# Ryukhaan/speech-to-video-mpp

Measured on AMD Instinct MI355X. Metric: synthesized 256×256 frames/sec/GPU (LNet+ENet path); 1/2/4/8-GPU scaling, higher is better.
Workload: dtype f32; 1 GPU; ENet(+LNet) forward, B=16 synthetic 256x256 crops + [1,80,16] mel windows -> 384x384 (models/ENet.py:82-139); crop=256, global_batch=16, batch_per_gpu=16, parallelism=frame-shard x1 (no data-path collective), graph=True, lanes=1, world_size_seen=1

## Files before the change

include/s2v.h:

```cpp
#ifndef S2V_H_
#define S2V_H_

#include <stddef.h>
#include <stdint.h>

#ifdef __cplusplus
extern "C" {
#endif

typedef void *s2v_stream_t;

enum {
    S2V_OK = 0,
    S2V_E_INVALID = -1,
    S2V_E_LAUNCH = -2,
    S2V_E_WORKSPACE = -3
};

enum {
    S2V_ACT_NONE = 0,
    S2V_ACT_RELU = 1,
    S2V_ACT_LRELU = 2,
    S2V_ACT_SIGMOID = 3,
    S2V_ACT_TANH = 4,
// ... 86 lines not shown

int s2v_modconv_demod_rows(const float *s, int batch, int s_ns, const int *rows, int nrows,
                           const float *wsq, float eps, float post, float *d, int d_ns,
                           s2v_stream_t stream);

int s2v_resize(const float *x, int n, int c, int ih, int iw, long long xsn, long long xsc, long long xsy,
               long long xsx, float *y, int oh, int ow, long long ysn, long long ysc, long long ysy,
               long long ysx, float scale_h, float scale_w, int mode, s2v_stream_t stream);

int s2v_torgb_up2(const float *x, int n, int h, int w, int c, int xcs, const float *wt, int kpad, const float *s,
                  int s_ns, const float *bias, const float *skip, int skcs, float *y, int ycs, s2v_stream_t stream);

typedef struct s2v_torgb_win {
    int fh, fw;
    int oy, ox;
    int sh, sw;
    int sy, sx;
    int nchw, cy, cx;
} s2v_torgb_win;
int s2v_torgb_up2_win(const float *x, int n, int h, int w, int c, int xcs, const float *wt, int kpad, const float *s,
                      int s_ns, const float *bias, const float *skip, int skcs, float *y, int ycs,
                      const s2v_torgb_win *win, s2v_stream_t stream);

typedef struct s2v_tapsum_win {
    int fh, fw;
    int oy, ox;
    int sy, sx;
} s2v_tapsum_win;
int s2v_tapsum_up2(const float *p, int n, int ph, int pw, int pcs, int cout, const float *noise, float pix_w,
                   const float *bias, float gain, int act, float alpha, float *y, int oh, int ow, int ycs,
                   const s2v_tapsum_win *win, s2v_stream_t stream);

int s2v_row_pack(const float *x, int n, int h, int w, int c, int xcs, int kw, int pw, float *y, int ycs,
                 s2v_stream_t stream);

int s2v_pad_reflect(const float *x, int n, int h, int w, int c, int xcs, int pt, int pb, int pl, int pr,
                    float *y, int ycs, s2v_stream_t stream);

int s2v_row_layernorm(const float *x, int rows, int dim, int xld, const float *weight, const float *bias,
                      float eps, float *y, int yld, s2v_stream_t stream);

int s2v_attention(const float *q, const float *k, const float *v, int batch, int heads, int tokens,
                  int dim_head, int ld_q, int ld_k, int ld_v, long long bs_q, long long bs_k, long long bs_v,
                  float scale, float *o, int ld_o, long long bs_o, s2v_stream_t stream);

int s2v_flow_warp(const float *flow, int n, int fh, int fw, int flow_cs, const float *src, int c, int h,
                  int w, long long ssn, long long ssc, long long ssy, long long ssx, float *y, int ycs,
                  s2v_stream_t stream);
int s2v_flow_warp_cat(const float *flow, int n, int fh, int fw, int flow_cs, const float *src, int c, int h,
                      int w, long long ssn, long long ssc, long long ssy, long long ssx, float *y, int ycs,
// ... 196 lines not shown
```

speech-to-video-mpp_amd/csrc/torch_launch.cpp:

```cpp
#include <ATen/ATen.h>
#include <ATen/hip/HIPContext.h>
#include <c10/core/DeviceGuard.h>
#include <torch/library.h>

#include <vector>

#include "../../include/s2v.h"

namespace {

using at::Tensor;
using OptT = c10::optional<Tensor>;

void *stream() { return (void *)at::hip::getCurrentHIPStream().stream(); }

void check(int rc, const char *what) { TORCH_CHECK(rc == 0, what, " failed (", rc, "): ", s2v_last_error()); }

bool has(const OptT &t) { return t && t->defined(); }

void same_dev(const Tensor &t, const at::Device &dev, const char *what) {
    TORCH_CHECK(t.is_cuda(), what, ": expected a HIP device tensor (the s2v ops have no CPU kernel)");
    TORCH_CHECK(t.device() == dev, what, ": on ", t.device(), ", the op's inputs are on ", dev);
}

// ... 677 lines not shown
        win.sy = (int)window[4]; win.sx = (int)window[5];
    }
    float *yp = nullptr;
    int ycs = 0;
    if (crop.empty()) {
        const NV yv = nhwc(y, dev, "torgb y");
        TORCH_CHECK(yv.n == xv.n && yv.h == xv.h && yv.w == xv.w && yv.c == 4, "torgb: y [N, H, W, 4] view expected");
        yp = yv.p; ycs = yv.cs;
    } else {
        f32(y, dev, "torgb y");
        TORCH_CHECK(crop[0] >= 0 && crop[1] >= 0 && 2 * crop[0] < xv.h && 2 * crop[1] < xv.w, "torgb crop: bad (cy, cx)");
        win.nchw = 1; win.cy = (int)crop[0]; win.cx = (int)crop[1];
        TORCH_CHECK(y.dim() == 4 && y.is_contiguous() && y.size(0) == xv.n && y.size(1) == 3 &&
                        y.size(2) == xv.h - 2 * win.cy && y.size(3) == xv.w - 2 * win.cx,
                    "torgb: contiguous NCHW y [N, 3, H - 2 cy, W - 2 cx] expected, got ", y.sizes());
        yp = y.data_ptr<float>();
    }
    check(s2v_torgb_up2_win(xv.p, xv.n, xv.h, xv.w, xv.c, xv.cs, wt.data_ptr<float>(), (int)wt.size(1),
                            s.data_ptr<float>(), s_ns, bp, kv.p, kv.cs, yp, ycs, &win, stream()),
          "s2v_torgb_up2");
}

void tapsum_up2_(const Tensor &p, const OptT &noise, double pix_w, const OptT &bias, double gain, int64_t act,
                 double alpha, const Tensor &y, at::IntArrayRef window) {
    const c10::DeviceGuard guard(p.device());
    const at::Device dev = p.device();
    const NV pv = nhwc(p, dev, "tapsum p"), yv = nhwc(y, dev, "tapsum y");
    TORCH_CHECK(yv.n == pv.n && pv.c == 9 * yv.c, "tapsum: p [N, PH, PW, 9 C] and y [N, OH, OW, C] views expected");
    TORCH_CHECK(window.empty() || window.size() == 6, "tapsum window: (fh, fw, oy, ox, sy, sx) or empty");
    s2v_tapsum_win win{};
    if (window.empty()) {
        TORCH_CHECK(yv.h == 2 * pv.h && yv.w == 2 * pv.w, "tapsum: y [N, 2 PH, 2 PW, C] expected");
    } else {
        for (int64_t v : window) TORCH_CHECK(v >= 0 && v < (1 << 29), "tapsum window: bad value ", v);
        win.fh = (int)window[0]; win.fw = (int)window[1]; win.oy = (int)window[2]; win.ox = (int)window[3];
        win.sy = (int)window[4]; win.sx = (int)window[5];
    }
    const float *np = vec(noise, dev, (int64_t)yv.n * yv.h * yv.w, "tapsum noise");
    const float *bp = vec(bias, dev, yv.c, "tapsum bias");
    check(s2v_tapsum_up2(pv.p, pv.n, pv.h, pv.w, pv.cs, yv.c, np, (float)pix_w, bp, (float)gain, (int)act, (float)alpha,
                         yv.p, yv.h, yv.w, yv.cs, &win, stream()),
          "s2v_tapsum_up2");
}

void flow_warp_(const Tensor &flow, const Tensor &src, const Tensor &y) {
    const c10::DeviceGuard guard(flow.device());
    const at::Device dev = flow.device();
    const NV fv = nhwc(flow, dev, "flow_warp flow"), yv = nhwc(y, dev, "flow_warp y");
    f32(src, dev, "flow_warp src");
    TORCH_CHECK(src.dim() == 4 && src.size(0) == fv.n && fv.c >= 2, "flow_warp: src [N, C, H, W], flow >= 2 channels");
    TORCH_CHECK(yv.n == fv.n && yv.h == src.size(2) && yv.w == src.size(3) && yv.c == src.size(1), "flow_warp: y shape");
    check(s2v_flow_warp(fv.p, fv.n, fv.h, fv.w, fv.cs, src.data_ptr<float>(), (int)src.size(1), (int)src.size(2),
                        (int)src.size(3), src.stride(0), src.stride(1), src.stride(2), src.stride(3), yv.p, yv.cs,
                        stream()),
          "s2v_flow_warp");
}

void flow_warp_cat_(const Tensor &flow, const Tensor &src, const Tensor &y) {
    const c10::DeviceGuard guard(flow.device());
    const at::Device dev = flow.device();
// ... 299 lines not shown
    m.def("group_end_(Tensor? ws, bool dry) -> int[]", &group_end_);
    m.def("gemm_kn_(Tensor a, Tensor b, Tensor(a!) out, int batch, int a_bs, int b_bs, int out_bs, Tensor? res, "
          "int res_bs, int act, float alpha, int prec, Tensor? ws, int force_tile, int force_splits, bool dry) -> int[]");
    m.def("split_weights_(Tensor w, Tensor(a!) out, int prec, float scale) -> ()");
    m.def("split_act_(Tensor x, Tensor(a!) out, int prec) -> ()");
    m.def("layernorm2d_(Tensor x, Tensor weight, Tensor bias, float eps, int act, float alpha, bool pool, "
          "Tensor? res, Tensor(a!) y, Tensor? ws) -> int");
    m.def("instnorm_(Tensor x, Tensor? gamma, Tensor? beta, float eps, int act, float alpha, Tensor? res, "
          "Tensor(a!) y, Tensor(b!)? pad_out, Tensor? ws) -> int");
    m.def("adain_params_(Tensor hid, int nhidden, Tensor w2t, Tensor bias, Tensor seg, Tensor(a!) out) -> ()");
    m.def("modconv_demod_(Tensor s, Tensor wsq, Tensor(a!) d, float eps, float post) -> ()");
    m.def("modconv_demod_rows_(Tensor s, Tensor rows, Tensor wsq, Tensor(a!) d, float eps, float post, "
          "int s_reach) -> ()");
    m.def("row_layernorm_(Tensor x, Tensor weight, Tensor bias, float eps, Tensor(a!) y) -> ()");
    m.def("attention_(Tensor q, Tensor k, Tensor v, Tensor(a!) out, int batch, int heads, int tokens, int dim_head, "
          "float scale) -> ()");
    m.def("resize_(Tensor x, int x_off, int[4] x_size, int[4] x_stride, Tensor(a!) y, int y_off, int[4] y_size, "
          "int[4] y_stride, float scale_h, float scale_w, int mode) -> ()");
    m.def("pad_reflect_(Tensor x, Tensor(a!) y, int[4] pads) -> ()");
    m.def("row_pack_(Tensor x, Tensor(a!) y, int kw, int pw) -> ()");
    m.def("torgb_up2_(Tensor x, Tensor wt, Tensor s, Tensor? bias, Tensor skip, Tensor(a!) y, int[] window, "
          "int[] crop) -> ()");
    m.def("tapsum_up2_(Tensor p, Tensor? noise, float pix_w, Tensor? bias, float gain, int act, float alpha, "
          "Tensor(a!) y, int[] window) -> ()");
    m.def("flow_warp_(Tensor flow, Tensor src, Tensor(a!) y) -> ()");
    m.def("flow_warp_cat_(Tensor flow, Tensor src, Tensor(a!) y) -> ()");
    m.def("fill_value_(Tensor(a!) y, float value) -> ()");
    m.def("gaussian_noise_(Tensor(a!) y, int seed, int offset, Tensor? ctr, int shift) -> ()");
    m.def("counter_add_(Tensor(a!) ctr, int inc) -> ()");
    m.def("rfft2_(Tensor x, Tensor tables, Tensor(a!) spec) -> ()");
    m.def("irfft2_(Tensor spec, Tensor tables, Tensor? res, Tensor(a!) y) -> ()");
    m.def("ffc_spec_fwd_(Tensor x_g, Tensor w1, float wt_scale, float x_scale, Tensor? scale, Tensor? shift, "
          "Tensor tables, Tensor(a!) t1, Tensor(b!) spec, Tensor? flag, int prec) -> ()");
    m.def("ffc_spec_inv_(Tensor spec, Tensor wfu, float wt_scale, float x_scale, Tensor? scale, Tensor? shift, "
          "Tensor tables, Tensor t1, Tensor(a!) u, Tensor? flag, int prec) -> ()");
    m.def("ffc_norm_(Tensor(c!) y, Tensor u, Tensor w2, float wt_scale, float x_scale, Tensor? gamma, Tensor? beta, "
          "float eps, int act, float alpha, Tensor? res, Tensor(a!) out, Tensor(b!)? pad_out, Tensor? flag, int prec) -> ()");
    m.def("eltwise_(Tensor x, Tensor? mul, Tensor? add, Tensor? bias, float a, int act, float alpha, float post, "
          "Tensor(a!) y) -> ()");
    m.def("fir2d_(Tensor x, Tensor kernel, Tensor(a!) y, int up, int down, int pad_y0, int pad_x0, float gain, "
          "Tensor? bias, int act, float alpha, float post) -> ()");
    m.def("lipsync_inputs_(Tensor src, Tensor? fake, Tensor(a!) ref_u8, Tensor(b!) face6, Tensor(c!) gt) -> ()");
    m.def("to_u8_(Tensor x, Tensor(a!) y, float lo, float hi, float scale, float offset) -> ()");
    m.def("mel_chunks_(Tensor mel, Tensor starts, int step, Tensor(a!) out) -> ()");
    m.def("melspectrogram_(Tensor wav, Tensor tables, bool pad_reflect, Tensor(a!) out) -> ()");
}

// ... 38 lines not shown
```

speech-to-video-mpp_amd/csrc/torgb.hip:

```cpp
#include "common.hpp"

namespace s2v {

__host__ __device__ __forceinline__ void up2_index(int dst, int in, int &i0, int &i1, float &l0, float &l1) {
    float src = 0.5f * ((float)dst + 0.5f) - 0.5f;
    if (src < 0.f) src = 0.f;
    i0 = (int)src;
    i1 = i0 + ((i0 < in - 1) ? 1 : 0);
    l1 = src - (float)i0;
    l0 = 1.f - l1;
}


struct TorgbGeo {
    int fsh, fsw;
    int oy, ox;
    int sh, sw;
    int sy, sx;
    int nchw, cy, cx;
};

template <int TPP, int PPT>
__global__ __launch_bounds__(256) void torgb_up2_kernel(const float *__restrict__ x, int C, int H, int W, int xcs,
                                                        const float *__restrict__ wt, int kpad,
// ... 97 lines not shown
    hi = i1;
}

struct TapsumGeo {
    int fh, fw;
    int ph, pw, sy, sx;
    int oh, ow, oy, ox;
    int k0, j0, ckh, ckw;
};

struct TapsumEpi {
    const float *noise;
    float pix_w;
    const float *bias;
    float gain;
    int act;
    float alpha;
    float *y;
    int ycs;
};

__device__ __forceinline__ constexpr float tapsum_w(int par, int ti) { return (par ^ ti) ? 0.25f : 0.75f; }

template <int DY, int DX>
__device__ __forceinline__ void tapsum_tap(const float *__restrict__ pt, const long long (&ro)[3], const long long (&co)[3],
                                           float4 (&acc)[2][2]) {
    constexpr int kLo[3] = {0, 0, 1}, kHi[3] = {1, 2, 2};
    float4 v[3][3];
#pragma unroll
    for (int si = 0; si < 3; ++si)
#pragma unroll
        for (int sj = 0; sj < 3; ++sj)
            if (si >= kLo[DY] && si <= kHi[DY] && sj >= kLo[DX] && sj <= kHi[DX])
                v[si][sj] = *(const float4 *)(pt + ro[si] + co[sj]);
#pragma unroll
    for (int a = 0; a < 2; ++a)
#pragma unroll
        for (int c = 0; c < 2; ++c) {
            const int bi = a + DY <= 1 ? 0 : 1, bj = c + DX <= 1 ? 0 : 1;
#pragma unroll
            for (int ti = 0; ti < 2; ++ti)
#pragma unroll
                for (int tj = 0; tj < 2; ++tj) {
                    const float cf = tapsum_w((a + DY) & 1, ti) * tapsum_w((c + DX) & 1, tj);
                    const float4 u = v[bi + ti][bj + tj];
                    acc[a][c].x = fmaf(cf, u.x, acc[a][c].x);
                    acc[a][c].y = fmaf(cf, u.y, acc[a][c].y);
                    acc[a][c].z = fmaf(cf, u.z, acc[a][c].z);
                    acc[a][c].w = fmaf(cf, u.w, acc[a][c].w);
                }
        }
}

__device__ __forceinline__ void tapsum_store(const TapsumEpi &e, const TapsumGeo &g, int b, int wr, int wc, int quad,
                                             float4 acc) {
    const long long pix = ((long long)b * g.oh + wr) * g.ow + wc;
    float4 bv = make_float4(0.f, 0.f, 0.f, 0.f);
    if (e.bias) bv = *(const float4 *)(e.bias + quad * 4);
    const float nz = e.noise ? e.pix_w * e.noise[pix] : 0.f;
    float4 r;
    r.x = apply_act(e.gain * acc.x + bv.x + nz, e.act, e.alpha);
    r.y = apply_act(e.gain * acc.y + bv.y + nz, e.act, e.alpha);
    r.z = apply_act(e.gain * acc.z + bv.z + nz, e.act, e.alpha);
    r.w = apply_act(e.gain * acc.w + bv.w + nz, e.act, e.alpha);
    *(float4 *)(e.y + pix * e.ycs + quad * 4) = r;
}

__global__ __launch_bounds__(256) void tapsum_up2_kernel(const float *__restrict__ P, int pcs, int cout, int quads,
                                                         long long items, TapsumEpi e, TapsumGeo g) {
    const long long item = (long long)xcd_block(blockIdx.x, gridDim.x) * 256 + threadIdx.x;
    if (item >= items) return;
    const int quad = (int)(item % quads);
    long long cell = item / quads;
    const int cj = (int)(cell % g.ckw);
    cell /= g.ckw;
    const int ck = (int)(cell % g.ckh);
    const int b = (int)(cell / g.ckh);
    const int k = g.k0 + ck, j = g.j0 + cj;
    const float *pb = P + (long long)b * g.ph * g.pw * pcs + quad * 4;
    if (k >= 1 && k <= g.fh - 2 && j >= 1 && j <= g.fw - 2) {
        long long ro[3], co[3];
#pragma unroll
        for (int s = 0; s < 3; ++s) {
            ro[s] = (long long)min(max(k + s - 1 - g.sy, 0), g.ph - 1) * g.pw * pcs;
            co[s] = (long long)min(max(j + s - 1 - g.sx, 0), g.pw - 1) * pcs;
        }
        float4 acc[2][2];
#pragma unroll
        for (int a = 0; a < 2; ++a)
#pragma unroll
            for (int c = 0; c < 2; ++c) acc[a][c] = make_float4(0.f, 0.f, 0.f, 0.f);
#pragma unroll 1
        for (int t = 0; t < 9; ++t) {
            const float *pt = pb + t * cout;
            switch (t) {
                case 0: tapsum_tap<0, 0>(pt, ro, co, acc); break;
                case 1: tapsum_tap<0, 1>(pt, ro, co, acc); break;
                case 2: tapsum_tap<0, 2>(pt, ro, co, acc); break;
                case 3: tapsum_tap<1, 0>(pt, ro, co, acc); break;
                case 4: tapsum_tap<1, 1>(pt, ro, co, acc); break;
                case 5: tapsum_tap<1, 2>(pt, ro, co, acc); break;
                case 6: tapsum_tap<2, 0>(pt, ro, co, acc); break;
                case 7: tapsum_tap<2, 1>(pt, ro, co, acc); break;
                default: tapsum_tap<2, 2>(pt, ro, co, acc); break;
            }
        }
#pragma unroll
        for (int a = 0; a < 2; ++a)
#pragma unroll
            for (int c = 0; c < 2; ++c) {
                const int wr = 2 * k + a - g.oy, wc = 2 * j + c - g.ox;
                if ((unsigned)wr < (unsigned)g.oh && (unsigned)wc < (unsigned)g.ow) tapsum_store(e, g, b, wr, wc, quad, acc[a][c]);
            }
        return;
    }
#pragma unroll 1
    for (int ac = 0; ac < 4; ++ac) {
        const int r = 2 * k + (ac >> 1), c = 2 * j + (ac & 1);
        const int wr = r - g.oy, wc = c - g.ox;
        if ((unsigned)wr >= (unsigned)g.oh || (unsigned)wc >= (unsigned)g.ow) continue;
        float4 acc = make_float4(0.f, 0.f, 0.f, 0.f);
#pragma unroll 1
        for (int t = 0; t < 9; ++t) {
            const int qy = r + t / 3 - 1, qx = c + t % 3 - 1;
            int i0, i1, j0, j1;
            float ly[2], lx[2];
            up2_index(qy, g.fh, i0, i1, ly[0], ly[1]);
            up2_index(qx, g.fw, j0, j1, lx[0], lx[1]);
            if (qy < 0 || qy >= 2 * g.fh) ly[0] = ly[1] = 0.f;
            if (qx < 0 || qx >= 2 * g.fw) lx[0] = lx[1] = 0.f;
            const long long rr[2] = {(long long)min(max(i0 - g.sy, 0), g.ph - 1) * g.pw * pcs,
                                     (long long)min(max(i1 - g.sy, 0), g.ph - 1) * g.pw * pcs};
            const long long cc[2] = {(long long)min(max(j0 - g.sx, 0), g.pw - 1) * pcs,
                                     (long long)min(max(j1 - g.sx, 0), g.pw - 1) * pcs};
            const float *pt = pb + t * cout;
#pragma unroll
            for (int ti = 0; ti < 2; ++ti)
#pragma unroll
                for (int tj = 0; tj < 2; ++tj) {
                    const float cf = ly[ti] * lx[tj];
                    const float4 u = *(const float4 *)(pt + rr[ti] + cc[tj]);
                    acc.x = fmaf(cf, u.x, acc.x);
                    acc.y = fmaf(cf, u.y, acc.y);
                    acc.z = fmaf(cf, u.z, acc.z);
                    acc.w = fmaf(cf, u.w, acc.w);
                }
        }
        tapsum_store(e, g, b, wr, wc, quad, acc);
    }
}

}

using namespace s2v;

extern "C" int s2v_tapsum_up2(const float *p, int n, int ph, int pw, int pcs, int cout, const float *noise, float pix_w,
                              const float *bias, float gain, int act, float alpha, float *y, int oh, int ow, int ycs,
                              const s2v_tapsum_win *win, s2v_stream_t stream) {
    S2V_REQUIRE(p && y && win && n > 0 && ph > 0 && pw > 0 && oh > 0 && ow > 0 && cout > 0, "tapsum_up2: bad args");
    S2V_REQUIRE(cout % 4 == 0, "tapsum_up2: Cout %d must be a multiple of 4 (16-byte channel accesses)", cout);
    S2V_REQUIRE(act == S2V_ACT_NONE || act == S2V_ACT_LRELU || act == S2V_ACT_RELU, "tapsum_up2: unknown act %d", act);
    const int fh = win->fh > 0 ? win->fh : ph, fw = win->fw > 0 ? win->fw : pw;
    S2V_REQUIRE(fh < (1 << 29) && fw < (1 << 29), "tapsum_up2: frame too large");
    S2V_REQUIRE(win->oy >= 0 && win->ox >= 0 && win->oy + (long long)oh <= 2LL * fh && win->ox + (long long)ow <= 2LL * fw,
                "tapsum_up2: the %dx%d output window at (%d, %d) leaves the %dx%d frame", oh, ow, win->oy, win->ox,
                2 * fh, 2 * fw);
    S2V_REQUIRE(win->sy >= 0 && win->sx >= 0 && win->sy + (long long)ph <= fh && win->sx + (long long)pw <= fw,
                "tapsum_up2: the %dx%d tap-product window at (%d, %d) leaves the %dx%d frame", ph, pw, win->sy, win->sx,
                fh, fw);
    int ylo, yhi, xlo, xhi;
    {
        const int qy0 = win->oy > 0 ? win->oy - 1 : 0, qy1 = win->oy + oh < 2 * fh ? win->oy + oh : 2 * fh - 1;
        const int qx0 = win->ox > 0 ? win->ox - 1 : 0, qx1 = win->ox + ow < 2 * fw ? win->ox + ow : 2 * fw - 1;
        up2_tap_range(qy0, qy1 - qy0 + 1, fh, ylo, yhi);
        up2_tap_range(qx0, qx1 - qx0 + 1, fw, xlo, xhi);
    }
    S2V_REQUIRE(ylo >= win->sy && yhi < win->sy + ph && xlo >= win->sx && xhi < win->sx + pw,
                "tapsum_up2: the output window at (%d, %d) reads tap-product rows %d..%d, columns %d..%d: outside the "
                "%dx%d tap-product window at (%d, %d)", win->oy, win->ox, ylo, yhi, xlo, xhi, ph, pw, win->sy, win->sx);
    S2V_REQUIRE(pcs % 4 == 0 && pcs >= 9LL * cout && ycs % 4 == 0 && ycs >= cout,
                "tapsum_up2: pixel pitches must hold 9 Cout / Cout channels and be multiples of 4");
    S2V_REQUIRE(((uintptr_t)p % 16) == 0 && ((uintptr_t)y % 16) == 0 && (!bias || ((uintptr_t)bias % 16) == 0),
                "tapsum_up2: 16-byte aligned p / y / bias");
    S2V_REQUIRE((long long)n * ph * pw * pcs < (1LL << 62) && (long long)n * oh * ow < (1LL << 40),
                "tapsum_up2: problem too large");
    const int k0 = win->oy >> 1, j0 = win->ox >> 1;
    const int ckh = ((win->oy + oh - 1) >> 1) - k0 + 1, ckw = ((win->ox + ow - 1) >> 1) - j0 + 1;
    const int quads = cout / 4;
    const long long items = (long long)n * ckh * ckw * quads;
    const long long blocks = (items + 255) / 256;
    S2V_REQUIRE(blocks < (1LL << 31), "tapsum_up2: grid too large");
    const TapsumGeo g{fh, fw, ph, pw, win->sy, win->sx, oh, ow, win->oy, win->ox, k0, j0, ckh, ckw};
    const TapsumEpi e{noise, noise ? pix_w : 0.f, bias, gain, act, alpha, y, ycs};
    tapsum_up2_kernel<<<(unsigned)blocks, 256, 0, (hipStream_t)stream>>>(p, pcs, cout, quads, items, e, g);
    return check_launch("tapsum_up2");
}

extern "C" int s2v_torgb_up2_win(const float *x, int n, int h, int w, int c, int xcs, const float *wt, int kpad,
                                 const float *s, int s_ns, const float *bias, const float *skip, int skcs, float *y,
                                 int ycs, const s2v_torgb_win *win, s2v_stream_t stream) {
    S2V_REQUIRE(x && wt && s && skip && y && win && n > 0 && h > 1 && w > 1 && c > 0, "torgb_up2: bad args");
    const int fh = win->fh > 0 ? win->fh : h, fw = win->fw > 0 ? win->fw : w;
    S2V_REQUIRE(fh % 2 == 0 && fw % 2 == 0, "torgb_up2: output frame %dx%d must be twice the skip frame", fh, fw);
    S2V_REQUIRE(win->oy >= 0 && win->ox >= 0 && win->oy + h <= fh && win->ox + w <= fw,
                "torgb_up2: the %dx%d output window at (%d, %d) leaves the %dx%d frame", h, w, win->oy, win->ox, fh, fw);
    S2V_REQUIRE(win->sh > 0 && win->sw > 0 && win->sy >= 0 && win->sx >= 0 && win->sy + win->sh <= fh / 2 &&
                    win->sx + win->sw <= fw / 2,
                "torgb_up2: the %dx%d skip window at (%d, %d) leaves the %dx%d skip frame", win->sh, win->sw, win->sy,
                win->sx, fh / 2, fw / 2);
    int ylo, yhi, xlo, xhi;
    up2_tap_range(win->oy, h, fh / 2, ylo, yhi);
    up2_tap_range(win->ox, w, fw / 2, xlo, xhi);
    S2V_REQUIRE(ylo >= win->sy && yhi < win->sy + win->sh && xlo >= win->sx && xhi < win->sx + win->sw,
                "torgb_up2: the output window at (%d, %d) reads skip rows %d..%d, columns %d..%d: outside the %dx%d "
                "skip window at (%d, %d)", win->oy, win->ox, ylo, yhi, xlo, xhi, win->sh, win->sw, win->sy, win->sx);
    S2V_REQUIRE(c % 32 == 0 && xcs % 4 == 0 && xcs >= c && kpad >= c && s_ns >= c && skcs % 4 == 0 && skcs >= 4,
                "torgb_up2: C %% 32 == 0, 4-channel skip, float4 pitches required");
// ... 37 lines not shown
```

speech-to-video-mpp_amd/engine/enet.py:

```python
from __future__ import annotations

import math
import os

import torch

from .. import ops
from ..ops import NHWC, ConvW
from .lnet import LNetEngine

LRELU = 0.2
OVERLAP = os.environ.get("S2V_ENET_OVERLAP", "1") == "1"
FUSED_TORGB = os.environ.get("S2V_ENET_FUSED_TORGB", "1") == "1"
POLY_UP = os.environ.get("S2V_ENET_POLY_UP", "1") == "1"
POLY_UP4 = os.environ.get("S2V_ENET_POLY_UP4", "0") == "1"
STYLE_GRID = os.environ.get("S2V_ENET_STYLE_GRID", "half")
ROWPACK0 = os.environ.get("S2V_ENET_ROWPACK0", "0") == "1"
FORK_AT = int(os.environ.get("S2V_ENET_FORK_AT", "0"))
PAUSE = tuple(int(v) for v in os.environ.get("S2V_ENET_PAUSE", "").split(":")) if os.environ.get("S2V_ENET_PAUSE") else None
PREMOD = os.environ.get("S2V_ENET_PREMOD", "1") == "1"
STACK_STRIPS = os.environ.get("S2V_ENET_STACK_STRIPS", "1") == "1"
RESUME_GRID = os.environ.get("S2V_ENET_RESUME_GRID", "")
CROP_TAIL = os.environ.get("S2V_ENET_CROP_TAIL", "1") == "1"
TAPSUM = os.environ.get("S2V_ENET_TAPSUM", "1") == "1"
TAP_TILE = int(os.environ.get("S2V_ENET_TAP_TILE", "9"))
OUT_CROP = 8


def crop_tail_cone(size: int, crop: int):
    f1, f2 = 2 * size, 4 * size
    lo, hi = crop, f2 - 1 - crop
    if crop < 3 or lo > hi:
        return None
    need = {"rgb1": (lo, hi), "conv4": (lo, hi), "conv3": (lo - 1, hi + 1)}
    p0, p1 = (lo - 1) // 2, (hi + 1) // 2
    need["conv2"] = (p0 - 1, p1 + 1)
    need["conv1"] = (p0 - 2, p1 + 2)
    need["rgb0"] = ((2 * lo - 1) // 4, (2 * hi - 1) // 4 + 1)
    win = {"conv1": (1, f1 - 2), "conv2": (2, f1 - 4), "rgb0": (2, f1 - 4), "conv3": (6, f2 - 12),
           "conv4": (7, f2 - 14), "rgb1": (7, f2 - 14)}
    for k, (a, b) in need.items():
        o, n = win[k]
        if n <= 0 or a < o or b > o + n - 1:
            return None
    return {"need": need, "win": win, "crop": crop - 7, "out": f2 - 2 * crop}


def style_grid(device) -> int:
# ... 177 lines not shown
                  (cur.t[:, :, 0:2], lambda t: t[:, :, 0:4], lambda t: t[:, :, 0:2], lambda t: t[:, :, 0:2]),
                  (cur.t[:, :, cur.w - 2:], lambda t: t[:, :, w2 - 4:], lambda t: t[:, :, 2:4],
                   lambda t: t[:, :, w2 - 2:]))
        for xs_t, nsel, ssel, ysel in strips:
            xs = NHWC(xs_t.contiguous())
            up = NHWC.empty(b, 2 * xs.h, 2 * xs.w, c, dev)
            ops.resize_nhwc(ctx, xs, up, scale_factor=2)
            ys = NHWC.empty(b, up.h, up.w, L.cout, dev)
            nz = None if noise is None else nsel(noise).contiguous()
            ops.modulated_conv2d(ctx, up, L.conv, ys, s, d, pix_add=nz, premod=wb.get("conv"), **kw)
            ysel(y.t).copy_(ssel(ys.t))
        return y

    def _crop_cone(self, size, out):
        L = self.layers
        if not (CROP_TAIL and POLY_UP and FUSED_TORGB) or L[0].conv4 is not None or L[0].rp is not None or \
                L[3].conv4 is None or L[1].conv4 is not None or L[4].conv4 is not None or L[2].cin % 32 or L[5].cin % 32:
            return None
        cone = crop_tail_cone(size, OUT_CROP)
        if cone is not None and tuple(out.shape[1:]) != (3, cone["out"], cone["out"]):
            return None
        return cone

    def _noise_window(self, ctx, L, idx, b, frame, origin, n, noises, ctr):
        if not L.noise_w:
            return None
        if noises is not None and noises[idx] is not None:
            plane = noises[idx].reshape(b, frame, frame)
        else:
            plane = torch.empty((b, frame, frame), device=self.device)
            ops.gaussian_noise(ctx, plane, self.noise_seed, idx << 36, ctr=ctr, shift=40)
            self.last_noises[idx] = plane
        return plane[:, origin: origin + n, origin: origin + n].contiguous()

    def _cropped_tail(self, ctx, cur: NHWC, s2, dtab, dall, wbs, noises, ctr, out, cone):
        dev, b, win = self.device, cur.n, cone["win"]
        f1, f2 = 2 * cur.h, 4 * cur.h
        L = self.layers
        kw = dict(act=ops.ACT_LRELU, alpha=LRELU, padding=(0, 0))

        def mod(j):
            sv = s2[:, self.mod_offs[j]: self.mod_offs[j] + L[j].cin]
            if L[j].is_rgb:
                return sv, None, {}
            idx = j - j // 3
            return sv, dtab.r0[idx], wbs.get(idx, {})

        x = NHWC.empty(b, f1, f1, cur.c, dev)
        ops.resize_nhwc(ctx, cur, x, scale_factor=2)
        for j, name in ((0, "conv1"), (1, "conv2")):
            o, n = win[name]
            s, r0, wb = mod(j)
            y = NHWC.empty(b, n, n, L[j].cout, dev)
            ops.modulated_conv2d(ctx, x, L[j].conv, y, s, dall[:, r0: r0 + L[j].cout], pix_w=L[j].noise_w or 0.0,
                                 pix_add=self._noise_window(ctx, L[j], j, b, f1, o, n, noises, ctr),
                                 premod=wb.get("conv"), **kw)
            x = y
        o, n = win["rgb0"]
        rgb0 = NHWC.empty(b, n, n, 4, dev)
        ops.torgb_up2(ctx, x, L[2].conv, mod(2)[0], cur, rgb0, frame=(f1, f1), origin=(o, o))
        o3, n3 = win["conv3"]
        s, r0, wb = mod(3)
        y = NHWC.empty(b, n3, n3, L[3].cout, dev)
        nz3 = self._noise_window(ctx, L[3], 2, b, f2, o3, n3, noises, ctr)
        if TAPSUM and L[3].conv9 is not None:
            o2 = win["conv2"][0]
            self._tapsum_styleconv(ctx, L[3], x, s, dall[:, r0: r0 + dtab.width[2]], wb.get("conv9"), nz3, y,
                                   frame=(f1, f1), origin=(o3, o3), src_origin=(o2, o2))
        else:
            ops.modulated_conv2d(ctx, x, L[3].conv4, y, s, dall[:, r0: r0 + dtab.width[2]], d2s=True,
                                 pix_w=L[3].noise_w or 0.0, pix_add=nz3, premod=wb.get("conv4"), **kw)
        o4, n4 = win["conv4"]
        s, r0, wb = mod(4)
        z = NHWC.empty(b, n4, n4, L[4].cout, dev)
        ops.modulated_conv2d(ctx, y, L[4].conv, z, s, dall[:, r0: r0 + L[4].cout], pix_w=L[4].noise_w or 0.0,
                             pix_add=self._noise_window(ctx, L[4], 3, b, f2, o4, n4, noises, ctr),
                             premod=wb.get("conv"), **kw)
        dst = out if out.is_contiguous() else torch.empty(out.shape, device=dev)
        ops.torgb_up2(ctx, z, L[5].conv, mod(5)[0], rgb0, dst, frame=(f2, f2), origin=(o4, o4), skip_origin=(o, o),
                      crop=(cone["crop"], cone["crop"]))
        if dst is not out:
            out.copy_(dst)

    def style_code(self, ctx, ref: torch.Tensor):
        st = self.style_begin(ctx, ref)
        self.style_down(ctx, st, len(self.down))
        return self.style_end(ctx, st)

    def style_begin(self, ctx, ref: torch.Tensor) -> dict:
        dev, b = self.device, ref.shape[0]
        x = NHWC.empty(b, 256, 256, 4, dev)
        ops.fill(ctx, x.t)
        ops.nchw_to_nhwc(ctx, ref, x.slice(0, 3))
        f = NHWC.empty(b, 256, 256, self.first.cout, dev)
        ops.conv2d(ctx, x, self.first, f, act=ops.ACT_LRELU, alpha=LRELU)
        return {"f": f, "i": 0}

    def style_down(self, ctx, st: dict, upto: int):
        f, b, dev = st["f"], st["f"].n, self.device
# ... 4 lines not shown
            ops.conv2d(ctx, f, c1, td, act=ops.ACT_LRELU, alpha=LRELU, pool=True)
            out = NHWC.empty(b, h // 2, w // 2, c2.cout, dev)
            ops.conv2d(ctx, f, sk, out)
            ops.conv2d(ctx, td, c2, out, act=ops.ACT_LRELU, alpha=LRELU, res=out, res_after=True)
            f = out
            st["i"] += 1
        st["f"] = f

    def style_end(self, ctx, st: dict):
        f, b, dev = st["f"], st["f"].n, self.device
        g = NHWC.empty(b, f.h, f.w, self.final_conv.cout, dev)
        ops.conv2d(ctx, f, self.final_conv, g, act=ops.ACT_LRELU, alpha=LRELU)
        style = NHWC.empty(b, 1, 1, self.final_linear.cout, dev)
        ops.conv2d(ctx, NHWC(g.t.view(b, 1, 1, -1)), self.final_linear, style)
        return style

    def forward(self, ctx, audio, face, gt, out: torch.Tensor, low: torch.Tensor, noises=None, aux=None):
        dev = self.device
        b = audio.shape[0]
        svec = NHWC.empty(b, 1, 1, self.mod.cout, dev)
        side = self._side(ctx) if OVERLAP else None
        cone = self._crop_cone(96 + 4, out)
        enc = {}

        def finish(sctx):
            enc["style"] = self.style_end(sctx, enc.pop("st"))
            ops.conv2d(sctx, enc["style"], self.mod, svec)
            enc["d"] = self._demods(sctx, svec.t.view(b, -1))
            if PREMOD:
                enc["wb"] = self._premodulate(sctx, svec.t.view(b, -1), enc["d"][0], enc["d"][1], b,
                                              strips=cone is None)

        def fork():
            sst, sctx = side
            sst.wait_stream(torch.cuda.current_stream(dev))
            with ops.x3_grid_cap(sctx, style_grid(dev)), ops.side_stream(sst, ctx.keep):
                enc["st"] = self.style_begin(sctx, face[:, 3:])
                self.style_down(sctx, enc["st"], PAUSE[0] if PAUSE else len(self.down))
                if not PAUSE:
                    finish(sctx)

        def resume():
            sst, sctx = side
            sst.wait_stream(torch.cuda.current_stream(dev))
            grid = int(RESUME_GRID) if RESUME_GRID else style_grid(dev)
            with ops.x3_grid_cap(sctx, grid), ops.side_stream(sst, ctx.keep):
                self.style_down(sctx, enc["st"], len(self.down))
                finish(sctx)

        on_level = None
        if side is not None:
            if FORK_AT:
                on_level = lambda h: fork() if h == FORK_AT and not enc else None
            else:
# ... 5 lines not shown
            ops.conv2d(ctx, enc["style"], self.mod, svec)
            enc["d"] = self._demods(ctx, svec.t.view(b, -1))
        x6 = NHWC.empty(b, 96, 96, 6, dev)
        ops.nchw_to_nhwc(ctx, face[:, :3], x6.slice(0, 3))
        ops.nchw_to_nhwc(ctx, gt, x6.slice(3, 3))
        lo = NHWC.empty(b, 96, 96, 4, dev)
        self.lnet.forward(ctx, audio, x6, lo, pad_rgb=True, on_level=on_level)
        if side is not None and not enc:
            fork()
        if side is not None and "st" in enc:
            resume()
        ops.nhwc_to_nchw(ctx, lo.slice(0, 3), low)
        if side is not None:
            torch.cuda.current_stream(dev).wait_stream(side[0])
        style, (dtab, dall) = enc["style"], enc["d"]
        s2 = svec.t.view(b, -1)
        if aux is not None:
            aux["style"] = style.t.view(b, -1)
        cur = NHWC.empty(b, 100, 100, 4, dev)
        ops.pad_reflect(ctx, lo, cur, (2, 2, 2, 2))
        skip = cur
        ctr = None
        self.last_noises = [None] * 4
        if noises is None and any(L.noise_w for L in self.layers):
            ctr = ctx.noise(id(self)).bump(ctx)
        if cone is not None:
            self._cropped_tail(ctx, cur, s2, dtab, dall, enc.get("wb", {}), noises, ctr, out, cone)
            return out, low
        for st in range(2):
            for li in range(2):
                L = self.layers[3 * st + li]
                off = self.mod_offs[3 * st + li]
                r0, wd = dtab.r0[2 * st + li], dtab.width[2 * st + li]
                if POLY_UP and L.conv4 is not None:
                    cur = self._poly_styleconv(ctx, L, cur, s2[:, off: off + L.cin], dall[:, r0: r0 + wd],
                                               2 * st + li, noises, ctr, wb=enc.get("wb", {}).get(2 * st + li))
                    continue
                x = cur
                if L.upsample:
                    x = NHWC.empty(b, 2 * cur.h, 2 * cur.w, cur.c, dev)
                    ops.resize_nhwc(ctx, cur, x, scale_factor=2)
                conv, cin = L.conv, L.cin
                if L.rp is not None:
                    xp = NHWC.empty(b, x.h, x.w, L.rp, dev)
                    ops.row_pack(ctx, x, xp, L.k, L.k // 2)
                    x, conv, cin = xp, L.conv.rowpack, L.rp
                d = dall[:, r0: r0 + L.cout]
                y = NHWC.empty(b, x.h, x.w, L.cout, dev)
                noise = None
                if L.noise_w:
# ... 22 lines not shown
```

speech-to-video-mpp_amd/ops.py:

```python
from __future__ import annotations

import contextlib
import ctypes
import math
import os
import threading
import weakref

import torch

from . import _lib, torch_ops
from ._lib import (ACT_GELU_TANH, ACT_LRELU, ACT_NONE, ACT_RELU, ACT_SIGMOID, ACT_TANH,
                   IN_DIRECT, IN_NEAREST_UP2, IN_TRANSPOSED, PAD_REFLECT, PAD_ZERO, PREC_BF16X3, PREC_F16, PREC_F16X3, PREC_F32,
                   check)

F32 = 4

_PRECISIONS = {"f16x3": PREC_F16X3, "bf16x3": PREC_BF16X3, "f32": PREC_F32, "f16": PREC_F16}
SPLIT_PRECISIONS = ("f16x3", "bf16x3")
PRECISION = os.environ.get("S2V_PRECISION", "f16x3")
if PRECISION not in _PRECISIONS:
    raise ValueError(f"S2V_PRECISION must be one of {sorted(_PRECISIONS)}, got {PRECISION!r}")


# ... 888 lines not shown
    assert skip.n == x.n and skip.c == 4
    if frame is None:
        assert origin == (0, 0) and skip_origin == (0, 0) and (2 * skip.h, 2 * skip.w) == (x.h, x.w)
        window = []
    else:
        window = [int(frame[0]), int(frame[1]), int(origin[0]), int(origin[1]), int(skip_origin[0]), int(skip_origin[1])]
    if crop is None:
        assert (y.n, y.h, y.w, y.c) == (x.n, x.h, x.w, 4)
        S2V.torgb_up2_(x.v, cw.wt, s, cw.shift, skip.v, y.v, window, [])
    else:
        assert tuple(y.shape) == (x.n, 3, x.h - 2 * crop[0], x.w - 2 * crop[1])
        S2V.torgb_up2_(x.v, cw.wt, s, cw.shift, skip.v, y, window, [int(crop[0]), int(crop[1])])
    return y


def up2_tap_window(origin: int, size: int, frame: int):
    q0, q1 = max(origin - 1, 0), min(origin + size, 2 * frame - 1)
    lo = int(max(0.5 * (q0 + 0.5) - 0.5, 0.0))
    hi = min(int(max(0.5 * (q1 + 0.5) - 0.5, 0.0)) + 1, frame - 1)
    return lo, hi - lo + 1


def tapsum_up2(ctx: Ctx, p: NHWC, y: NHWC, *, bias=None, pix_add=None, pix_w=0.0, gain=1.0, act=ACT_NONE, alpha=0.0,
               frame=None, origin=(0, 0), src_origin=(0, 0)):
    assert p.n == y.n and p.c == 9 * y.c, "tapsum_up2: p carries nine tap blocks of y's channels"
    if frame is None:
        assert origin == (0, 0) and src_origin == (0, 0) and (y.h, y.w) == (2 * p.h, 2 * p.w)
        window = []
    else:
        window = [int(frame[0]), int(frame[1]), int(origin[0]), int(origin[1]), int(src_origin[0]), int(src_origin[1])]
    if pix_add is not None:
        assert tuple(pix_add.shape) == (y.n, y.h, y.w) and pix_add.is_contiguous()
    S2V.tapsum_up2_(p.v, pix_add, float(pix_w), bias, float(gain), int(act), float(alpha), y.v, window)
    return y


def row_pack(ctx: Ctx, x: NHWC, y: NHWC, kw: int, pw: int):
    S2V.row_pack_(x.v, y.v, kw, pw)
    return y


def pad_reflect(ctx: Ctx, x: NHWC, y: NHWC, pads):
    S2V.pad_reflect_(x.v, y.v, list(pads))
    return y


def row_layernorm(ctx: Ctx, x: torch.Tensor, weight, bias, y: torch.Tensor, eps=1e-5):
    S2V.row_layernorm_(x, weight, bias, eps, y)
    return y


def attention(ctx: Ctx, q: torch.Tensor, k: torch.Tensor, v: torch.Tensor, out: torch.Tensor, *, batch, heads,
              tokens, dim_head=64, scale=None):
    scale = dim_head ** -0.5 if scale is None else scale
    S2V.attention_(q, k, v, out, batch, heads, tokens, dim_head, scale)
    return out
# ... 148 lines not shown
```

Before: 741.0 frames/s.

## Compute two tapsum cells per thread and pre-draw noise planes on side stream

The tapsum upsample kernel now lets each thread process a run of two adjacent cells. The overlapping column loads of the 3x3 source neighbourhood are shared between them, which cuts redundant global loads and index math but raises register use. A separate change draws the gaussian noise planes and their cropped windows during the overlapped side-stream encode phase, moving that work off the main critical path. The cost is extra allocations and full-plane generation before cropping.

```diff
diff --git a/include/s2v.h b/include/s2v.h
--- a/include/s2v.h
+++ b/include/s2v.h
@@ -132,10 +132,13 @@
                       int s_ns, const float *bias, const float *skip, int skcs, float *y, int ycs,
                       const s2v_torgb_win *win, s2v_stream_t stream);
 
+#define S2V_TAPSUM_RUN 0
+#define S2V_TAPSUM_CELL 1
 typedef struct s2v_tapsum_win {
     int fh, fw;
     int oy, ox;
     int sy, sx;
+    int variant;
 } s2v_tapsum_win;
 int s2v_tapsum_up2(const float *p, int n, int ph, int pw, int pcs, int cout, const float *noise, float pix_w,
                    const float *bias, float gain, int act, float alpha, float *y, int oh, int ow, int ycs,
diff --git a/speech-to-video-mpp_amd/csrc/torch_launch.cpp b/speech-to-video-mpp_amd/csrc/torch_launch.cpp
--- a/speech-to-video-mpp_amd/csrc/torch_launch.cpp
+++ b/speech-to-video-mpp_amd/csrc/torch_launch.cpp
@@ -723,7 +723,7 @@
 }
 
 void tapsum_up2_(const Tensor &p, const OptT &noise, double pix_w, const OptT &bias, double gain, int64_t act,
-                 double alpha, const Tensor &y, at::IntArrayRef window) {
+                 double alpha, const Tensor &y, at::IntArrayRef window, int64_t variant) {
     const c10::DeviceGuard guard(p.device());
     const at::Device dev = p.device();
     const NV pv = nhwc(p, dev, "tapsum p"), yv = nhwc(y, dev, "tapsum y");
@@ -737,6 +737,8 @@
         win.fh = (int)window[0]; win.fw = (int)window[1]; win.oy = (int)window[2]; win.ox = (int)window[3];
         win.sy = (int)window[4]; win.sx = (int)window[5];
     }
+    TORCH_CHECK(variant >= 0 && variant <= 1, "tapsum variant: bad value ", variant);
+    win.variant = (int)variant;
     const float *np = vec(noise, dev, (int64_t)yv.n * yv.h * yv.w, "tapsum noise");
     const float *bp = vec(bias, dev, yv.c, "tapsum bias");
     check(s2v_tapsum_up2(pv.p, pv.n, pv.h, pv.w, pv.cs, yv.c, np, (float)pix_w, bp, (float)gain, (int)act, (float)alpha,
@@ -1082,7 +1084,7 @@
     m.def("torgb_up2_(Tensor x, Tensor wt, Tensor s, Tensor? bias, Tensor skip, Tensor(a!) y, int[] window, "
           "int[] crop) -> ()");
     m.def("tapsum_up2_(Tensor p, Tensor? noise, float pix_w, Tensor? bias, float gain, int act, float alpha, "
-          "Tensor(a!) y, int[] window) -> ()");
+          "Tensor(a!) y, int[] window, int variant) -> ()");
     m.def("flow_warp_(Tensor flow, Tensor src, Tensor(a!) y) -> ()");
     m.def("flow_warp_cat_(Tensor flow, Tensor src, Tensor(a!) y) -> ()");
     m.def("fill_value_(Tensor(a!) y, float value) -> ()");
diff --git a/speech-to-video-mpp_amd/csrc/torgb.hip b/speech-to-video-mpp_amd/csrc/torgb.hip
--- a/speech-to-video-mpp_amd/csrc/torgb.hip
+++ b/speech-to-video-mpp_amd/csrc/torgb.hip
@@ -143,17 +143,8 @@
 
 __device__ __forceinline__ constexpr float tapsum_w(int par, int ti) { return (par ^ ti) ? 0.25f : 0.75f; }
 
-template <int DY, int DX>
-__device__ __forceinline__ void tapsum_tap(const float *__restrict__ pt, const long long (&ro)[3], const long long (&co)[3],
-                                           float4 (&acc)[2][2]) {
-    constexpr int kLo[3] = {0, 0, 1}, kHi[3] = {1, 2, 2};
-    float4 v[3][3];
-#pragma unroll
-    for (int si = 0; si < 3; ++si)
-#pragma unroll
-        for (int sj = 0; sj < 3; ++sj)
-            if (si >= kLo[DY] && si <= kHi[DY] && sj >= kLo[DX] && sj <= kHi[DX])
-                v[si][sj] = *(const float4 *)(pt + ro[si] + co[sj]);
+template <int DY, int DX, int W>
+__device__ __forceinline__ void tapsum_fma(const float4 (&v)[3][W], int c0, float4 (&acc)[2][2]) {
 #pragma unroll
     for (int a = 0; a < 2; ++a)
 #pragma unroll
@@ -164,13 +155,28 @@
 #pragma unroll
                 for (int tj = 0; tj < 2; ++tj) {
                     const float cf = tapsum_w((a + DY) & 1, ti) * tapsum_w((c + DX) & 1, tj);
-                    const float4 u = v[bi + ti][bj + tj];
+                    const float4 u = v[bi + ti][c0 + bj + tj];
                     acc[a][c].x = fmaf(cf, u.x, acc[a][c].x);
                     acc[a][c].y = fmaf(cf, u.y, acc[a][c].y);
                     acc[a][c].z = fmaf(cf, u.z, acc[a][c].z);
                     acc[a][c].w = fmaf(cf, u.w, acc[a][c].w);
                 }
         }
+}
+
+template <int DY, int DX, int R>
+__device__ __forceinline__ void tapsum_tap(const float *__restrict__ pt, const long long (&ro)[3],
+                                           const long long (&co)[R + 2], float4 (&acc)[R][2][2]) {
+    constexpr int kLo[3] = {0, 0, 1}, kHi[3] = {1, 2, 2};
+    float4 v[3][R + 2];
+#pragma unroll
+    for (int si = 0; si < 3; ++si)
+#pragma unroll
+        for (int sj = 0; sj < R + 2; ++sj)
+            if (si >= kLo[DY] && si <= kHi[DY] && sj >= kLo[DX] && sj <= kHi[DX] + R - 1)
+                v[si][sj] = *(const float4 *)(pt + ro[si] + co[sj]);
+#pragma unroll
+    for (int i = 0; i < R; ++i) tapsum_fma<DY, DX, R + 2>(v, i, acc[i]);
 }
 
 __device__ __forceinline__ void tapsum_store(const TapsumEpi &e, const TapsumGeo &g, int b, int wr, int wc, int quad,
@@ -187,54 +193,8 @@
     *(float4 *)(e.y + pix * e.ycs + quad * 4) = r;
 }
 
-__global__ __launch_bounds__(256) void tapsum_up2_kernel(const float *__restrict__ P, int pcs, int cout, int quads,
-                                                         long long items, TapsumEpi e, TapsumGeo g) {
-    const long long item = (long long)xcd_block(blockIdx.x, gridDim.x) * 256 + threadIdx.x;
-    if (item >= items) return;
-    const int quad = (int)(item % quads);
-    long long cell = item / quads;
-    const int cj = (int)(cell % g.ckw);
-    cell /= g.ckw;
-    const int ck = (int)(cell % g.ckh);
-    const int b = (int)(cell / g.ckh);
-    const int k = g.k0 + ck, j = g.j0 + cj;
-    const float *pb = P + (long long)b * g.ph * g.pw * pcs + quad * 4;
-    if (k >= 1 && k <= g.fh - 2 && j >= 1 && j <= g.fw - 2) {
-        long long ro[3], co[3];
-#pragma unroll
-        for (int s = 0; s < 3; ++s) {
-            ro[s] = (long long)min(max(k + s - 1 - g.sy, 0), g.ph - 1) * g.pw * pcs;
-            co[s] = (long long)min(max(j + s - 1 - g.sx, 0), g.pw - 1) * pcs;
-        }
-        float4 acc[2][2];
-#pragma unroll
-        for (int a = 0; a < 2; ++a)
-#pragma unroll
-            for (int c = 0; c < 2; ++c) acc[a][c] = make_float4(0.f, 0.f, 0.f, 0.f);
-#pragma unroll 1
-        for (int t = 0; t < 9; ++t) {
-            const float *pt = pb + t * cout;
-            switch (t) {
-                case 0: tapsum_tap<0, 0>(pt, ro, co, acc); break;
-                case 1: tapsum_tap<0, 1>(pt, ro, co, acc); break;
-                case 2: tapsum_tap<0, 2>(pt, ro, co, acc); break;
-                case 3: tapsum_tap<1, 0>(pt, ro, co, acc); break;
-                case 4: tapsum_tap<1, 1>(pt, ro, co, acc); break;
-                case 5: tapsum_tap<1, 2>(pt, ro, co, acc); break;
-                case 6: tapsum_tap<2, 0>(pt, ro, co, acc); break;
-                case 7: tapsum_tap<2, 1>(pt, ro, co, acc); break;
-                default: tapsum_tap<2, 2>(pt, ro, co, acc); break;
-            }
-        }
-#pragma unroll
-        for (int a = 0; a < 2; ++a)
-#pragma unroll
-            for (int c = 0; c < 2; ++c) {
-                const int wr = 2 * k + a - g.oy, wc = 2 * j + c - g.ox;
-                if ((unsigned)wr < (unsigned)g.oh && (unsigned)wc < (unsigned)g.ow) tapsum_store(e, g, b, wr, wc, quad, acc[a][c]);
-            }
-        return;
-    }
+__device__ __forceinline__ void tapsum_border_cell(const float *__restrict__ pb, int pcs, int cout, const TapsumEpi &e,
+                                                   const TapsumGeo &g, int b, int k, int j, int quad) {
 #pragma unroll 1
     for (int ac = 0; ac < 4; ++ac) {
         const int r = 2 * k + (ac >> 1), c = 2 * j + (ac & 1);
@@ -271,6 +231,82 @@
     }
 }
 
+template <int R>
+__device__ __forceinline__ void tapsum_interior(const float *__restrict__ pb, int pcs, int cout, const TapsumEpi &e,
+                                                const TapsumGeo &g, int b, int k, int j, int quad) {
+    long long ro[3], co[R + 2];
+#pragma unroll
+    for (int s = 0; s < 3; ++s) ro[s] = (long long)min(max(k + s - 1 - g.sy, 0), g.ph - 1) * g.pw * pcs;
+#pragma unroll
+    for (int s = 0; s < R + 2; ++s) co[s] = (long long)min(max(j + s - 1 - g.sx, 0), g.pw - 1) * pcs;
+    float4 acc[R][2][2];
+#pragma unroll
+    for (int i = 0; i < R; ++i)
+#pragma unroll
+        for (int a = 0; a < 2; ++a)
+#pragma unroll
+            for (int c = 0; c < 2; ++c) acc[i][a][c] = make_float4(0.f, 0.f, 0.f, 0.f);
+#pragma unroll 1
+    for (int t = 0; t < 9; ++t) {
+        const float *pt = pb + t * cout;
+        switch (t) {
+            case 0: tapsum_tap<0, 0, R>(pt, ro, co, acc); break;
+            case 1: tapsum_tap<0, 1, R>(pt, ro, co, acc); break;
+            case 2: tapsum_tap<0, 2, R>(pt, ro, co, acc); break;
+            case 3: tapsum_tap<1, 0, R>(pt, ro, co, acc); break;
+            case 4: tapsum_tap<1, 1, R>(pt, ro, co, acc); break;
+            case 5: tapsum_tap<1, 2, R>(pt, ro, co, acc); break;
+            case 6: tapsum_tap<2, 0, R>(pt, ro, co, acc); break;
+            case 7: tapsum_tap<2, 1, R>(pt, ro, co, acc); break;
+            default: tapsum_tap<2, 2, R>(pt, ro, co, acc); break;
+        }
+    }
+#pragma unroll
+    for (int i = 0; i < R; ++i)
+#pragma unroll
+        for (int a = 0; a < 2; ++a)
+#pragma unroll
+            for (int c = 0; c < 2; ++c) {
+                const int wr = 2 * k + a - g.oy, wc = 2 * (j + i) + c - g.ox;
+                if ((unsigned)wr < (unsigned)g.oh && (unsigned)wc < (unsigned)g.ow)
+                    tapsum_store(e, g, b, wr, wc, quad, acc[i][a][c]);
+            }
+}
+
+template <int R>
+__global__ __launch_bounds__(256) void tapsum_up2_kernel(const float *__restrict__ P, int pcs, int cout, int quads,
+                                                         int runs, long long items, TapsumEpi e, TapsumGeo g) {
+    const long long item = (long long)xcd_block(blockIdx.x, gridDim.x) * 256 + threadIdx.x;
+    if (item >= items) return;
+    const int quad = (int)(item % quads);
+    long long rest = item / quads;
+    const int cj0 = (int)(rest % runs) * R;
+    rest /= runs;
+    const int ck = (int)(rest % g.ckh);
+    const int b = (int)(rest / g.ckh);
+    const int k = g.k0 + ck, jr = g.j0 + cj0;
+    const int ncell = min(R, g.ckw - cj0);
+    const float *pb = P + (long long)b * g.ph * g.pw * pcs + quad * 4;
+    const bool rowint = k >= 1 && k <= g.fh - 2;
+    if (R > 1 && rowint && ncell == R && jr >= 1 && jr + R - 1 <= g.fw - 2) {
+        tapsum_interior<R>(pb, pcs, cout, e, g, b, k, jr, quad);
+        return;
+    }
+#pragma unroll 1
+    for (int i = 0; i < ncell; ++i) {
+        const int j = jr + i;
+        if (rowint && j >= 1 && j <= g.fw - 2) tapsum_interior<1>(pb, pcs, cout, e, g, b, k, j, quad);
+        else tapsum_border_cell(pb, pcs, cout, e, g, b, k, j, quad);
+    }
+}
+
+template <int R>
+static void launch_tapsum(const float *p, int pcs, int cout, int n, const TapsumEpi &e, const TapsumGeo &g, hipStream_t st) {
+    const int quads = cout / 4, runs = (g.ckw + R - 1) / R;
+    const long long items = (long long)n * g.ckh * runs * quads;
+    tapsum_up2_kernel<R><<<(unsigned)((items + 255) / 256), 256, 0, st>>>(p, pcs, cout, quads, runs, items, e, g);
+}
+
 }
 
 using namespace s2v;
@@ -307,13 +343,13 @@
                 "tapsum_up2: problem too large");
     const int k0 = win->oy >> 1, j0 = win->ox >> 1;
     const int ckh = ((win->oy + oh - 1) >> 1) - k0 + 1, ckw = ((win->ox + ow - 1) >> 1) - j0 + 1;
-    const int quads = cout / 4;
-    const long long items = (long long)n * ckh * ckw * quads;
-    const long long blocks = (items + 255) / 256;
-    S2V_REQUIRE(blocks < (1LL << 31), "tapsum_up2: grid too large");
+    S2V_REQUIRE(win->variant == S2V_TAPSUM_RUN || win->variant == S2V_TAPSUM_CELL, "tapsum_up2: unknown kernel variant %d",
+                win->variant);
+    S2V_REQUIRE((long long)n * ckh * ckw * (cout / 4) / 256 < (1LL << 31) - 1, "tapsum_up2: grid too large");
     const TapsumGeo g{fh, fw, ph, pw, win->sy, win->sx, oh, ow, win->oy, win->ox, k0, j0, ckh, ckw};
     const TapsumEpi e{noise, noise ? pix_w : 0.f, bias, gain, act, alpha, y, ycs};
-    tapsum_up2_kernel<<<(unsigned)blocks, 256, 0, (hipStream_t)stream>>>(p, pcs, cout, quads, items, e, g);
+    if (win->variant == S2V_TAPSUM_CELL) launch_tapsum<1>(p, pcs, cout, n, e, g, (hipStream_t)stream);
+    else launch_tapsum<2>(p, pcs, cout, n, e, g, (hipStream_t)stream);
     return check_launch("tapsum_up2");
 }
 
diff --git a/speech-to-video-mpp_amd/engine/enet.py b/speech-to-video-mpp_amd/engine/enet.py
--- a/speech-to-video-mpp_amd/engine/enet.py
+++ b/speech-to-video-mpp_amd/engine/enet.py
@@ -24,6 +24,7 @@
 CROP_TAIL = os.environ.get("S2V_ENET_CROP_TAIL", "1") == "1"
 TAPSUM = os.environ.get("S2V_ENET_TAPSUM", "1") == "1"
 TAP_TILE = int(os.environ.get("S2V_ENET_TAP_TILE", "9"))
+PRE_NOISE = os.environ.get("S2V_ENET_PRE_NOISE", "1") == "1"
 OUT_CROP = 8
 
 
@@ -247,9 +248,30 @@
             return None
         return cone
 
-    def _noise_window(self, ctx, L, idx, b, frame, origin, n, noises, ctr):
+    def _draw_noises(self, sctx, lane, b, size, cone):
+        ctr = lane.noise(id(self)).bump(sctx)
+        pre = []
+        for idx, (j, name) in enumerate(((0, "conv1"), (1, "conv2"), (3, "conv3"), (4, "conv4"))):
+            if not self.layers[j].noise_w:
+                pre.append(None)
+                continue
+            frame = (2 if idx < 2 else 4) * size
+            plane = ops.empty((b, frame, frame), self.device)
+            ops.gaussian_noise(sctx, plane, self.noise_seed, idx << 36, ctr=ctr, shift=40)
+            win = None
+            if cone is not None:
+                o, n = cone["win"][name]
+                win = ops.empty((b, n, n), self.device)
+                win.copy_(plane[:, o: o + n, o: o + n])
+            pre.append((plane, win))
+        return pre
+
+    def _noise_window(self, ctx, L, idx, b, frame, origin, n, noises, ctr, pre=None):
         if not L.noise_w:
             return None
+        if pre is not None:
+            assert tuple(pre[idx][1].shape) == (b, n, n)
+            return pre[idx][1]
         if noises is not None and noises[idx] is not None:
             plane = noises[idx].reshape(b, frame, frame)
         else:
@@ -258,7 +280,7 @@
             self.last_noises[idx] = plane
         return plane[:, origin: origin + n, origin: origin + n].contiguous()
 
-    def _cropped_tail(self, ctx, cur: NHWC, s2, dtab, dall, wbs, noises, ctr, out, cone):
+    def _cropped_tail(self, ctx, cur: NHWC, s2, dtab, dall, wbs, noises, ctr, out, cone, pre=None):
         dev, b, win = self.device, cur.n, cone["win"]
         f1, f2 = 2 * cur.h, 4 * cur.h
         L = self.layers
@@ -278,7 +300,7 @@
             s, r0, wb = mod(j)
             y = NHWC.empty(b, n, n, L[j].cout, dev)
             ops.modulated_conv2d(ctx, x, L[j].conv, y, s, dall[:, r0: r0 + L[j].cout], pix_w=L[j].noise_w or 0.0,
-                                 pix_add=self._noise_window(ctx, L[j], j, b, f1, o, n, noises, ctr),
+                                 pix_add=self._noise_window(ctx, L[j], j, b, f1, o, n, noises, ctr, pre),
                                  premod=wb.get("conv"), **kw)
             x = y
         o, n = win["rgb0"]
@@ -287,7 +309,7 @@
         o3, n3 = win["conv3"]
         s, r0, wb = mod(3)
         y = NHWC.empty(b, n3, n3, L[3].cout, dev)
-        nz3 = self._noise_window(ctx, L[3], 2, b, f2, o3, n3, noises, ctr)
+        nz3 = self._noise_window(ctx, L[3], 2, b, f2, o3, n3, noises, ctr, pre)
         if TAPSUM and L[3].conv9 is not None:
             o2 = win["conv2"][0]
             self._tapsum_styleconv(ctx, L[3], x, s, dall[:, r0: r0 + dtab.width[2]], wb.get("conv9"), nz3, y,
@@ -299,7 +321,7 @@
         s, r0, wb = mod(4)
         z = NHWC.empty(b, n4, n4, L[4].cout, dev)
         ops.modulated_conv2d(ctx, y, L[4].conv, z, s, dall[:, r0: r0 + L[4].cout], pix_w=L[4].noise_w or 0.0,
-                             pix_add=self._noise_window(ctx, L[4], 3, b, f2, o4, n4, noises, ctr),
+                             pix_add=self._noise_window(ctx, L[4], 3, b, f2, o4, n4, noises, ctr, pre),
                              premod=wb.get("conv"), **kw)
         dst = out if out.is_contiguous() else torch.empty(out.shape, device=dev)
         ops.torgb_up2(ctx, z, L[5].conv, mod(5)[0], rgb0, dst, frame=(f2, f2), origin=(o4, o4), skip_origin=(o, o),
@@ -350,6 +372,7 @@
         side = self._side(ctx) if OVERLAP else None
         cone = self._crop_cone(96 + 4, out)
         enc = {}
+        pre_noise = PRE_NOISE and side is not None and noises is None and any(L.noise_w for L in self.layers)
 
         def finish(sctx):
             enc["style"] = self.style_end(sctx, enc.pop("st"))
@@ -358,6 +381,8 @@
             if PREMOD:
                 enc["wb"] = self._premodulate(sctx, svec.t.view(b, -1), enc["d"][0], enc["d"][1], b,
                                               strips=cone is None)
+            if pre_noise:
+                enc["noise"] = self._draw_noises(sctx, ctx, b, 96 + 4, cone)
 
         def fork():
             sst, sctx = side
@@ -409,10 +434,15 @@
         skip = cur
         ctr = None
         self.last_noises = [None] * 4
-        if noises is None and any(L.noise_w for L in self.layers):
+        pre = enc.get("noise")
+        if pre is not None:
+            self.last_noises = [None if pn is None else pn[0] for pn in pre]
+            if cone is None:
+                noises = self.last_noises
+        elif noises is None and any(L.noise_w for L in self.layers):
             ctr = ctx.noise(id(self)).bump(ctx)
         if cone is not None:
-            self._cropped_tail(ctx, cur, s2, dtab, dall, enc.get("wb", {}), noises, ctr, out, cone)
+            self._cropped_tail(ctx, cur, s2, dtab, dall, enc.get("wb", {}), noises, ctr, out, cone, pre)
             return out, low
         for st in range(2):
             for li in range(2):
diff --git a/speech-to-video-mpp_amd/ops.py b/speech-to-video-mpp_amd/ops.py
--- a/speech-to-video-mpp_amd/ops.py
+++ b/speech-to-video-mpp_amd/ops.py
@@ -934,8 +934,10 @@
 
 
 def tapsum_up2(ctx: Ctx, p: NHWC, y: NHWC, *, bias=None, pix_add=None, pix_w=0.0, gain=1.0, act=ACT_NONE, alpha=0.0,
-               frame=None, origin=(0, 0), src_origin=(0, 0)):
+               frame=None, origin=(0, 0), src_origin=(0, 0), variant=None):
     assert p.n == y.n and p.c == 9 * y.c, "tapsum_up2: p carries nine tap blocks of y's channels"
+    if variant is None:
+        variant = int(os.environ.get("S2V_TAPSUM_VARIANT", "0"))
     if frame is None:
         assert origin == (0, 0) and src_origin == (0, 0) and (y.h, y.w) == (2 * p.h, 2 * p.w)
         window = []
@@ -943,7 +945,8 @@
         window = [int(frame[0]), int(frame[1]), int(origin[0]), int(origin[1]), int(src_origin[0]), int(src_origin[1])]
     if pix_add is not None:
         assert tuple(pix_add.shape) == (y.n, y.h, y.w) and pix_add.is_contiguous()
-    S2V.tapsum_up2_(p.v, pix_add, float(pix_w), bias, float(gain), int(act), float(alpha), y.v, window)
+    S2V.tapsum_up2_(p.v, pix_add, float(pix_w), bias, float(gain), int(act), float(alpha), y.v, window,
+                    int(variant))
     return y
 
 
```

Result: no change. 750.1 frames/s (median of 5 runs) (+1.2%).
